# dcjones/polee

Measured on AMD Instinct MI355X. Metric: approx-lik VI iters/sec, higher is better.
Workload: dtype f32

## Files before the change

### include/polee_hip_debug.h

```cpp
#ifndef POLEE_HIP_DEBUG_H
#define POLEE_HIP_DEBUG_H

#include "polee_hip.h"

#ifdef __cplusplus
extern "C" {
#endif

polee_status polee_debug_ptt_plan(const int32_t *node_parent_idxs, const int32_t *node_js, int32_t N,
                                  uint32_t *tour_code, int32_t *tour_tgt, int32_t *leaf_tid,
                                  int32_t *lo, int32_t *mid, int32_t *hi1, int32_t *max_depth);

typedef struct polee_psell_debug polee_psell_debug;
typedef struct {
    int64_t m, n, nnz, num_slices, num_tiles, padded_nnz, num_empty_rows;
    int64_t data_bytes, dict_len;
    int32_t max_row_nnz, max_tile_cols;
    const uint8_t *data;
    const uint32_t *slice_off;
    const uint32_t *tile_slice;
    const uint32_t *tile_dict;
    const uint32_t *dict;
    const uint32_t *row_order;
    const float *slice_ks;
    const uint8_t *slice_flags;
    int64_t num_tiles_a;
    int64_t num_tiles_a1;
    int64_t num_tiles_a1m;
    int64_t num_tiles_a2;
    const uint8_t *slice_w;
    int64_t num_tiles_s;
    int64_t stream_rows[8], stream_nnz[8], stream_bytes[8];
    int64_t csr_num_rows;
    const uint32_t *csr_rowptr;
    const uint32_t *csr_col;
    const float *csr_val;
    const uint32_t *csr_rows;
    int64_t single_num_rows;
    const uint32_t *single_rows;
    const float *single_cnt;
    double single_logsum;
} polee_psell_view;
polee_status polee_debug_psell_build(int64_t m, int64_t n, const void *colptr, int colptr_bytes,
                                     const uint32_t *rowval, const float *nzval,
                                     const int64_t *ks_or_null, polee_psell_debug **out);
polee_status polee_debug_psell_build_device(polee_ctx *ctx, int64_t m, int64_t n, const void *colptr, int colptr_bytes,
                                            const uint32_t *rowval, const float *nzval, const int64_t *ks_or_null,
                                            int device_stages, polee_psell_debug **out);
polee_status polee_debug_psell_view(const polee_psell_debug *p, polee_psell_view *view);
void polee_debug_psell_free(polee_psell_debug *p);

void polee_debug_device_cache_poison(int64_t *checked_blocks, int64_t *bad_blocks, int64_t *bad_words);

polee_status polee_debug_loglik_force_mixed(polee_loglik *ll, int on);

int64_t polee_debug_regression_num_stats(const polee_regression *reg);
polee_status polee_debug_regression_data_pass(polee_regression *reg, const float *noise, float *stats);
polee_status polee_debug_regression_prior_pass(polee_regression *reg, const float *stats, float *loss,
                                               float *grad_or_null);

polee_status polee_debug_comm_allreduce_ms(polee_comm *comm, int64_t count, int32_t reps, double *ms_avg);

polee_status polee_debug_fast_log(polee_ctx *ctx, const double *x, int64_t count, double *out);
polee_status polee_debug_fast_exp(polee_ctx *ctx, const double *x, int64_t count, double *out);

polee_status polee_debug_approx_node_terms(polee_approx *ap, double *tpair, float *bp);

polee_status polee_vi_debug_set_draw_split(polee_vi *vi, int32_t dpw_fwd, int32_t dpw_bwd, int32_t dpw_update);

polee_status polee_debug_gibbs_assignments(polee_gibbs *g, int32_t chain, int32_t *z);

polee_status polee_debug_binomial(polee_ctx *ctx, const int64_t *N, const double *p, int64_t count, uint64_t seed, int64_t *out);

polee_status polee_debug_kmer_edges_count(polee_ctx *ctx_or_null, int64_t n, const uint64_t *sketches, int64_t *count);
polee_status polee_debug_kmer_edges_fill(polee_ctx *ctx_or_null, int64_t n, const uint64_t *sketches, int64_t capacity,
                                         uint32_t *u, uint32_t *v, uint32_t *mat, uint32_t *empt);
polee_status polee_debug_kmer_round_select(polee_ctx *ctx_or_null, int64_t num_nodes, int64_t E, const uint32_t *u, const uint32_t *v,
                                           const uint64_t *key, uint8_t *merged_flags, int32_t *order);

#ifdef __cplusplus
}
#endif
#endif
```

### polee_amd/csrc/debug.cpp

```cpp
#include <algorithm>
#include <memory>

#include "../../include/polee_hip_debug.h"
#include "loglik_internal.hpp"
#include "ptt_internal.hpp"
#include "psell_device.hpp"

using namespace polee;

struct polee_psell_debug {
    PsellHost h;
};

extern "C" {

polee_status polee_debug_ptt_plan(const int32_t *node_parent_idxs, const int32_t *node_js, int32_t N,
                                  uint32_t *tour_code, int32_t *tour_tgt, int32_t *leaf_tid, int32_t *lo,
                                  int32_t *mid, int32_t *hi1, int32_t *max_depth)
{
    if (!node_parent_idxs || !node_js) return fail(nullptr, POLEE_ERR_BAD_ARG, "null argument");
    std::vector<int32_t> l, r, f;
    std::string err = children_from_parents(node_parent_idxs, node_js, N, l, r, f);
    PttPlan pl;
    if (err.empty()) err = build_ptt_plan(l.data(), r.data(), f.data(), N, pl);
// ... 79 lines not shown
        if (needs_host) {
            if (runs_on_device) POLEE_TRY(psell_device_runs_to_host(ctx, DR, R));
            if ((err = psell_stage2(m, n, rowptr.data(), col.data(), val.data(), ks, R, p->h, W)) != "") return bad(err);
        } else {
            rows_on_device = true;
        }
    } else {
        if (runs_on_device) POLEE_TRY(psell_device_runs_to_host(ctx, DR, R));
        if ((err = psell_stage2(m, n, rowptr.data(), col.data(), val.data(), ks, R, p->h, W)) != "") return bad(err);
    }
    if (device_stages & 4) {
        if (!rows_on_device) {
            DW.Nr = W.rows.size();
            DW.npat = W.pat_ptr.size() - 1;
            const size_t b[7] = {0, (size_t)p->h.rows_a1, (size_t)p->h.rows_a1m, (size_t)p->h.rows_a2, (size_t)p->h.rows_a, (size_t)p->h.rows_s, W.rows.size()};
            for (int q = 0; q < 7; ++q) DW.bounds[q] = b[q];
            POLEE_TRY(DW.rows.upload(ctx, W.rows.data(), W.rows.size()));
            POLEE_TRY(DW.run_end.upload(ctx, W.run_end.data(), W.run_end.size()));
            POLEE_TRY(DW.gid.upload(ctx, W.row_gid.data(), W.row_gid.size()));
            POLEE_TRY(DW.form.upload(ctx, W.row_form.data(), W.row_form.size()));
            POLEE_TRY(DW.pat_ptr.upload(ctx, W.pat_ptr.data(), W.pat_ptr.size()));
            POLEE_TRY(DW.pat_col.upload(ctx, W.pat_col.data(), W.pat_col.size()));
        }
        PsellDevOut D;
        POLEE_TRY(psell_device_stage3(ctx, X, DW.view(), p->h, D, true));
    } else {
        if (rows_on_device) POLEE_TRY(psell_device_rows_to_host(ctx, DW, p->h, W));
        if ((err = psell_stage3(m, n, rowptr.data(), col.data(), val.data(), ks, W, p->h)) != "") return bad(err);
    }
    *out = p.release();
    return POLEE_OK;
}

polee_status polee_debug_psell_build(int64_t m, int64_t n, const void *colptr, int colptr_bytes, const uint32_t *rowval,
                                     const float *nzval, const int64_t *ks, polee_psell_debug **out)
{
    return guarded(nullptr, "polee_debug_psell_build", [&] { return debug_psell_build_impl(m, n, colptr, colptr_bytes, rowval, nzval, ks, out); });
}
polee_status polee_debug_psell_build_device(polee_ctx *ctx, int64_t m, int64_t n, const void *colptr, int colptr_bytes,
                                            const uint32_t *rowval, const float *nzval, const int64_t *ks, int device_stages,
                                            polee_psell_debug **out)
{
    return guarded(ctx, "polee_debug_psell_build_device",
                   [&] { return debug_psell_build_device_impl(ctx, m, n, colptr, colptr_bytes, rowval, nzval, ks, device_stages, out); });
}

polee_status polee_debug_psell_view(const polee_psell_debug *p, polee_psell_view *v)
{
    if (!p || !v) return fail(nullptr, POLEE_ERR_BAD_ARG, "null argument");
    const PsellHost &h = p->h;
    v->m = h.m; v->n = h.n; v->nnz = h.nnz;
    v->num_slices = h.num_slices; v->num_tiles = h.num_tiles; v->padded_nnz = h.padded_nnz;
    v->num_empty_rows = h.empty_rows;
    v->data_bytes = (int64_t)h.data.size(); v->dict_len = (int64_t)h.dict.size();
    v->max_row_nnz = h.max_row; v->max_tile_cols = h.max_tile_cols;
    v->data = h.data.data(); v->slice_off = h.slice_off.data(); v->tile_slice = h.tile_slice.data();
    v->tile_dict = h.tile_dict.data(); v->dict = h.dict.data(); v->row_order = h.row_order.data();
    v->slice_ks = h.slice_ks.empty() ? nullptr : h.slice_ks.data();
    v->slice_flags = h.slice_flags.data();
    v->num_tiles_a = h.num_tiles_a;
    v->num_tiles_a1 = h.num_tiles_a1;
    v->num_tiles_a1m = h.num_tiles_a1m;
    v->num_tiles_a2 = h.num_tiles_a2;
    v->num_tiles_s = h.num_tiles_s;
    v->slice_w = h.slice_w.data();
    for (int i = 0; i < 8; ++i) v->stream_rows[i] = v->stream_nnz[i] = v->stream_bytes[i] = 0;
    v->csr_num_rows = (int64_t)h.csr_rows.size();
    v->csr_rowptr = h.csr_rowptr.data();
    v->csr_col = h.csr_col.data();
    v->csr_val = h.csr_val.data();
    v->csr_rows = h.csr_rows.data();
    v->single_num_rows = (int64_t)h.single_rows.size();
    v->single_rows = h.single_rows.data();
    v->single_cnt = h.single_cnt.empty() ? nullptr : h.single_cnt.data();
    v->single_logsum = h.single_logsum;
    for (int i = 0; i < PSELL_NSTREAMS; ++i) {
        v->stream_rows[i] = h.stream_rows[i];
        v->stream_nnz[i] = h.stream_nnz[i];
        v->stream_bytes[i] = h.stream_bytes[i];
    }
    return POLEE_OK;
}

void polee_debug_psell_free(polee_psell_debug *p) { delete p; }

}
```

### polee_amd/csrc/loglik.hip

```cpp
#include "loglik_stream.hpp"

#include <algorithm>
#include <cmath>
#include <queue>

namespace polee {

template <int K>
__device__ inline void scatter_runs(int c, float (&q)[K], float *gw, int lane)
{
    const int c0 = __builtin_amdgcn_readfirstlane(c);
    if (__all(c == c0)) {
        float *gr = gw + c0 * K;
        wave_sum_to_lane63_n<K>(q);
        if (lane == 63) {
#pragma unroll
            for (int k = 0; k < K; ++k) atomicAdd(gr + k, q[k]);
        }
        return;
    }
    const int cprev = __builtin_amdgcn_update_dpp(-1, c, 0x138 , 0xf, 0xf, false);
    const unsigned long long heads = __ballot(c != cprev);
    const unsigned long long upto = lane == 63 ? ~0ull : ((2ull << lane) - 1ull);
    const int dist = lane - (63 - __clzll(heads & upto));
// ... 286 lines not shown
    double ls[PSELL_MAX_K];
#pragma unroll
    for (int k = 0; k < PSELL_MAX_K; ++k) ls[k] = 0.0;
    if (c != 0.0f) {
        const float *xr = x + (size_t)j * K;
        float *gr = g + (size_t)j * K;
#pragma unroll
        for (int k = 0; k < PSELL_MAX_K; ++k)
            if (k < K) {
                const float xv = xr[k];
                if (g) gr[k] += c / xv;
                if (part) ls[k] = (double)c * log((double)xv);
            }
    }
    if (!part) return;
#pragma unroll
    for (int k = 0; k < PSELL_MAX_K; ++k) {
        double v = ls[k];
#pragma unroll
        for (int d = 32; d >= 1; d >>= 1) v += __shfl_down(v, d, 64);
        if ((threadIdx.x & 63) == 0) sm[threadIdx.x >> 6][k] = v;
    }
    __syncthreads();
    if (threadIdx.x < K) part[(size_t)blockIdx.x * K + threadIdx.x] = ((sm[0][threadIdx.x] + sm[1][threadIdx.x]) + sm[2][threadIdx.x]) + sm[3][threadIdx.x];
}
__global__ void single_lp_finish_kernel(const double *__restrict__ part, int nblocks, int K, double logsum, double *__restrict__ lp)
{
    const int k = threadIdx.x;
    if (k >= K) return;
    double s = logsum;
    for (int b = 0; b < nblocks; ++b) s += part[(size_t)b * K + k];
    lp[k] += s;
}

static const double TILE_COST_FIXED[PSELL_NSTREAMS] = {8700.0, 9000.0, 8700.0, 5000.0, 2000.0, 2000.0};
static const double TILE_COST_PER_KIB[PSELL_NSTREAMS] = {350.0, 750.0, 310.0, 1400.0, 3100.0, 3100.0};
static double slices_cost(const PsellHost &h, int stream, uint32_t sa, uint32_t sb)
{
    const double kib = 0.125 * (double)((h.slice_off[sb] & PSELL_OFF_MASK) - (h.slice_off[sa] & PSELL_OFF_MASK));
    static const bool old_cost = getenv("POLEE_OLD_COST") != nullptr;
    if (old_cost) return (kib * 1024.0 + 4096.0) * (stream == PSELL_A2 || stream == PSELL_A2M ? 1.5 : 1.0);
    return TILE_COST_FIXED[stream] + TILE_COST_PER_KIB[stream] * kib;
}
static void wave_cuts(const PsellHost &h, int64_t t, uint32_t s0, uint32_t s1, uint32_t cut[3])
{
    cut[0] = cut[1] = cut[2] = s1;
    if (t >= h.num_tiles_s) return;
    static const bool bytes_cut = getenv("POLEE_BYTES_CUT") != nullptr;
    const int nw = h.stream_of_tile(t) != PSELL_A2M ? 4 : 2;
    static const char *cut_env = getenv("POLEE_CUT_MODEL");
    static double cm[3] = {0, 0, 0};
    static const bool cut_custom = cut_env && sscanf(cut_env, "%lf,%lf,%lf", &cm[0], &cm[1], &cm[2]) == 3;
    auto cost = [&](uint32_t sl) {
        const int w = h.slice_w[sl];
        if (bytes_cut) return 512.0 + 128.0 * (double)((h.slice_off[sl + 1] & PSELL_OFF_MASK) - (h.slice_off[sl] & PSELL_OFF_MASK));
        if (h.stream_of_tile(t) == PSELL_BN) return 6.0 * w + 4.0;
        if (cut_custom) {
            const double ng = (double)((w + 3) / 4);
            const bool cont = (h.slice_flags[sl] & 2) != 0 && sl > s0;
            return cm[0] + cm[1] * ng + (cont ? 0.0 : cm[2] * (1.0 + ng));
        }
        return 4.0 * ((w + 3) / 4) + (w <= 8 ? 8.0 : 16.0 * ((w + 15) / 16)) + 10.0;
    };
    double total = 0.0;
    for (uint32_t sl = s0; sl < s1; ++sl) total += cost(sl);
    double acc = 0.0;
    int wv = 1;
    for (uint32_t sl = s0; sl < s1 && wv < nw; ++sl) {
        acc += cost(sl);
        while (wv < nw && (acc >= total * wv / nw || sl + 1 - (wv == 1 ? s0 : cut[wv - 2]) >= 63u)) cut[wv++ - 1] = sl + 1;
    }
    if (s1 - (nw > 1 ? cut[nw - 2] : s0) > 63u) {
        const uint32_t per = (s1 - s0 + (uint32_t)nw - 1) / (uint32_t)nw;
        for (int q = 1; q < nw; ++q) cut[q - 1] = std::min(s1, s0 + per * (uint32_t)q);
    }
}

void loglik_prepare_tiles(polee_loglik *ll)
{
    const PsellHost &h = ll->host;
    ll->tile_cost.assign((size_t)h.num_tiles, 0.0f);
    for (int64_t t = 0; t < h.num_tiles; ++t)
        ll->tile_cost[(size_t)t] = (float)slices_cost(h, h.stream_of_tile(t), h.tile_slice[t], h.tile_slice[t + 1]);
    ll->tile_cut.assign((size_t)3 * h.num_tiles, 0u);
    for (int64_t t = 0; t < h.num_tiles; ++t) wave_cuts(h, t, h.tile_slice[t], h.tile_slice[t + 1], &ll->tile_cut[(size_t)3 * t]);
}

polee_status loglik_ensure_schedule(polee_loglik *ll, int G)
{
    if (ll->sched_grid == G && ll->d_sched.p) return POLEE_OK;
    const PsellHost &h = ll->host;
    std::vector<uint32_t> order;
    order.reserve((size_t)h.num_tiles_s);
    for (int64_t t = 0; t < h.num_tiles_s; ++t) order.push_back((uint32_t)t);
    std::stable_sort(order.begin(), order.end(), [&](uint32_t a, uint32_t b) { return ll->tile_cost[a] > ll->tile_cost[b]; });
    std::vector<std::vector<uint32_t>> lists((size_t)G);
    {
        typedef std::pair<double, int> Load;
        std::priority_queue<Load, std::vector<Load>, std::greater<Load>> heap;
        for (int b = 0; b < G; ++b) heap.push(Load(0.0, b));
        for (uint32_t t : order) {
            Load l = heap.top();
            heap.pop();
            lists[(size_t)l.second].push_back(t);
            l.first += (double)ll->tile_cost[t];
            heap.push(l);
        }
    }
    size_t rounds = 0;
    for (auto &l : lists) rounds = std::max(rounds, l.size());
    std::vector<PosDesc> sched((rounds + 3) * (size_t)G);
    for (auto &d : sched) {
        d = PosDesc();
        d.tile = POS_NONE;
    }
    for (int b = 0; b < G; ++b) {
        std::vector<uint32_t> big, small;
        for (uint32_t t : lists[b]) (h.stream_of_tile(t) != PSELL_A2 && h.stream_of_tile(t) != PSELL_A2M ? big : small).push_back(t);
        const size_t n = big.size() + small.size();
        size_t ib = 0, is = 0;
        for (size_t j = 0; j < n; ++j) {
            const size_t want = ((j + 1 + (size_t)(b % 3)) * small.size()) / (n + 2);
            const bool take_small = (is < small.size()) && (ib >= big.size() || is < want);
            const uint32_t t = take_small ? small[is++] : big[ib++];
            PosDesc &d = sched[j * (size_t)G + (size_t)b];
            d.tile = t;
            d.s0 = h.tile_slice[t];
            d.s1 = h.tile_slice[t + 1];
            d.d0 = h.tile_dict[t];
            d.L = h.tile_cols[t];
            d.c1 = ll->tile_cut[(size_t)3 * t];
            d.c2 = ll->tile_cut[(size_t)3 * t + 1];
            d.c3 = ll->tile_cut[(size_t)3 * t + 2];
        }
    }
    POLEE_TRY(ll->d_sched.upload(ll->ctx, sched));
    ll->sched_grid = G;
    if (!ll->d_sched_dyn.p) {
        std::vector<uint32_t> dorder(order);
        {
            static const bool plain = getenv("POLEE_DYN_PLAIN_ORDER") != nullptr;
            std::vector<double> key((size_t)h.num_tiles_s, 0.0);
            size_t cnt[PSELL_NSTREAMS] = {}, seen[PSELL_NSTREAMS] = {};
            for (uint32_t t : order) ++cnt[h.stream_of_tile(t)];
            for (uint32_t t : order) {
                const int st = h.stream_of_tile(t);
                key[t] = ((double)seen[st] + 0.5) / (double)cnt[st];
                ++seen[st];
            }
            if (!plain) std::stable_sort(dorder.begin(), dorder.end(), [&](uint32_t a, uint32_t b) { return key[a] < key[b]; });
        }
        std::vector<PosDesc> plist;
        plist.reserve(dorder.size());
        for (size_t i = 0; i < dorder.size(); ++i) {
            const uint32_t t = dorder[i];
            PosDesc d = PosDesc();
            d.tile = t;
            d.s0 = h.tile_slice[t];
            d.s1 = h.tile_slice[t + 1];
            d.d0 = h.tile_dict[t];
            d.L = h.tile_cols[t];
            d.c1 = ll->tile_cut[(size_t)3 * t];
            d.c2 = ll->tile_cut[(size_t)3 * t + 1];
            d.c3 = ll->tile_cut[(size_t)3 * t + 2];
            plist.push_back(d);
        }
        ll->dyn_positions = plist.size();
        std::vector<PosDesc> dynl(plist.size() + (size_t)4 * 4 * 256 + 64);
// ... 346 lines not shown
```

### polee_amd/csrc/loglik_internal.hpp

```cpp
#pragma once
#include "common.hpp"
#include "psell_slice.hpp"

namespace polee {

constexpr int PSELL_MAX_TILE_COLS = 1024;
constexpr int PSELL_TILE_COLS_TARGET = 128;
constexpr int PSELL_DICT_ALIGN = 4;
constexpr int PSELL_TILE_SLICES_A1 = 64;
constexpr int PSELL_TILE_SLICES_A2 = 32;
constexpr int PSELL_TILE_SLICES_B = 16;
constexpr int PSELL_MAX_K = 8;
constexpr int PSELL_NARROW_MAX = 16;
constexpr int PSELL_WIDE_MAX = 32;
constexpr int PSELL_MIXED_NARROW_MAX = 15;
constexpr int PSELL_TILE_SLICES_A2M = 16;
constexpr int PSELL_TILE_SLICES_BN = 64;
constexpr uint32_t PSELL_PACK_CHUNK = 1u << 11;
constexpr uint32_t PSELL_MIXED_SEG_ROWS = 1u << 12;
constexpr double PSELL_PACK_WIDE_RESERVE = 32768.0;
constexpr int PSELL_MIN_UNIFORM_ROWS = 32;
constexpr int PSELL_MIN_UNION_ROWS = 1;

struct PosDesc {
// ... 62 lines not shown
    const uint32_t *csr_col;
    const uint32_t *index_of;
    bool singles_in_g;
};
}

struct polee_xbuild;
namespace polee {
polee_status xbuild_device_view(const polee_xbuild *xb, polee_ctx **ctx, int64_t *rows, int64_t *n, const uint64_t **tcolptr,
                                const uint32_t **trowval, const float **tnzval);
}

struct polee_devx {
    polee_ctx *ctx = nullptr;
    int64_t m = 0, n = 0;
    uint64_t nnz = 0;
    polee::DevBuf<uint64_t> cp;
    polee::DevBuf<uint32_t> rowval;
    polee::DevBuf<float> nzval;
};

struct polee_loglik {
    polee_ctx *ctx = nullptr;
    int refs = 1;
    int64_t m = 0, n = 0, nnz = 0;
    bool has_ks = false;
    bool device_built = false;
    bool force_mixed = false;
    bool xwin_ready = false;
    const double *side_part = nullptr;
    int side_nparts = 0;
    double *side_out = nullptr;
    bool side_done = false;
    polee::PsellHost host;
    polee::DevBuf<uint8_t> d_data;
    polee::DevBuf<uint32_t> d_slice_off, d_tile_slice, d_tile_dict, d_dict;
    polee::DevBuf<float> d_slice_ks;
    polee::DevBuf<uint32_t> d_csr_rowptr;
    polee::DevBuf<uint32_t> d_csr_col;
    polee::DevBuf<float> d_csr_val, d_csr_ks;
    int64_t csr_rows = 0, csr_nnz = 0;
    polee::DevBuf<float> d_single_cnt;
    polee::DevBuf<double> d_single_part;
    bool has_singles = false;
    const polee::LoglikRemap *cur_remap = nullptr;
    polee::DevBuf<float> d_xwin;
    polee::DevBuf<polee::PosDesc> d_sched;
    int sched_grid = 0;
    polee::DevBuf<polee::PosDesc> d_sched_dyn;
    polee::DevBuf<unsigned int> d_dyn_ctr;
    size_t dyn_pad = 0;
    size_t dyn_positions = 0;
    uint32_t dyn_base = 0;
    std::vector<float> tile_cost;
    std::vector<uint32_t> tile_cut;
    int64_t dict_len = 0;
    int occ_cache[polee::PSELL_MAX_K + 1][2][2][2] = {};
    bool deterministic = false;
    polee::DevBuf<float> d_gwin;
    polee::DevBuf<double> d_lpwin;
    polee::DevBuf<uint32_t> d_tslot_ptr, d_tslot, d_theavy;
    polee::DevBuf<float> d_x_rows, d_x_aos, d_g_aos;
    polee::DevBuf<double> d_g_rows, d_lp;
    bool profile = false;
    int prof_every = 1;
    uint64_t prof_tick = 0;
    hipEvent_t cur_e0 = nullptr, cur_e1 = nullptr;
    hipEvent_t cur_p0 = nullptr, cur_p1 = nullptr;
    std::vector<hipEvent_t> prof_events;
    size_t prof_used = 0;
    int64_t prof_launches = 0;
    double prof_ms_total = 0.0, prof_pass_ms_total = 0.0;
    polee_status profile_collect();
};

namespace polee {
void loglik_retain(polee_loglik *ll);
void loglik_release(polee_loglik *ll);
polee_status loglik_eval_device(polee_loglik *ll, const float *d_x, int K, float *d_g, double *d_lp, bool xwin_ready = false,
                                const LoglikRemap *remap = nullptr);
constexpr int SINGLE_THREADS = 256;
constexpr uint32_t GWIN_HEAVY = 32;
void loglik_prepare_tiles(polee_loglik *ll);
polee_status loglik_ensure_schedule(polee_loglik *ll, int G);
std::string csc_to_csr(int64_t m, int64_t n, const void *colptr, int colptr_bytes, const uint32_t *rowval, const float *nzval,
                       BVec<uint64_t> &rowptr, RawVec<uint32_t> &col, RawVec<float> &val);
}
```

### polee_amd/csrc/loglik_stream.hpp

```cpp
#pragma once
#include "loglik_internal.hpp"
#include "wave.hpp"

#include <type_traits>

namespace polee {

typedef float f32x2 __attribute__((ext_vector_type(2)));
typedef float f32x4 __attribute__((ext_vector_type(4)));
typedef const __attribute__((address_space(3))) float *lds_cfp;
typedef __attribute__((address_space(3))) float *lds_fp;
typedef const __attribute__((address_space(3))) f32x2 *lds_cf2p;
typedef const __attribute__((address_space(3))) uint16_t *lds_cu16p;
__device__ inline float lds_f(uint32_t a) { return *reinterpret_cast<lds_cfp>((uintptr_t)a); }

template <int CTRL, int ROW_MASK>
__device__ inline float dpp_mov0(float v)
{
    return __int_as_float(__builtin_amdgcn_update_dpp(0, __float_as_int(v), CTRL, ROW_MASK, 0xf, true));
}

__device__ inline float fast_weight(float ksv, float s)
{
    return s > 0.0f ? ksv * __builtin_amdgcn_rcpf(s) : 0.0f;
// ... 641 lines not shown
{
    constexpr int WMAX = PSELL_NARROW_MAX;
    static_assert(WMAX == 16, "four groups of four transcripts");
    constexpr int KG = (K + 3) / 4;
    const int lane = wave_lane();
    const uint32_t ring_lds = lds_addr(ring);
    const uint32_t xw_lds = lds_addr(xw), gw_lds = lds_addr(gw);
    const int j = lane & 3, b = lane >> 2;
    const uint32_t j4 = 4u * (uint32_t)j;
    uint32_t lc1[4];
#pragma unroll
    for (int u = 0; u < 4; ++u) lc1[u] = ring_lds + ((uint32_t)(lane ^ u) << 2);
    const uint32_t j256 = 256u * (uint32_t)j;

    f32x4 acc[4][KG];
    float xq[8][KG];
#pragma unroll
    for (int g = 0; g < 4; ++g)
#pragma unroll
        for (int kg = 0; kg < KG; ++kg) acc[g][kg] = f32x4{0.f, 0.f, 0.f, 0.f};
#pragma unroll
    for (int t = 0; t < 8; ++t)
#pragma unroll
        for (int kg = 0; kg < KG; ++kg) xq[t][kg] = 0.0f;
    uint32_t xav = aux_lds;
    uint32_t gaq = aux_lds + 32u;
    int pend_w = 0;
    int run_w = 0;
    QuadLp<KG> lp;
    f32x4 floorq = f32x4{ROWSUM_FLOOR, ROWSUM_FLOOR, ROWSUM_FLOOR, ROWSUM_FLOOR};
    asm volatile("" : "+v"(floorq));

    auto flush = [&]() {
        quad_flush_spread<K, 0>(acc[0], gaq, lane, j, dbg);
        if (pend_w > 4) quad_flush_spread<K, 1>(acc[1], gaq, lane, j, dbg);
        if (pend_w > 8) quad_flush_spread<K, 2>(acc[2], gaq, lane, j, dbg);
        if (pend_w > 12) quad_flush_spread<K, 3>(acc[3], gaq, lane, j, dbg);
        pend_w = 0;
    };

    RingCursor<RB, true> rc(ws, ring_lds, extras, lc1[0]);
    uint32_t e_next = (uint32_t)__builtin_amdgcn_readlane((int)ws.ent, 0);
    for (int si = 0; si < ws.nsl; ++si) {
        const uint32_t e0 = e_next;
        const uint32_t e1 = (uint32_t)__builtin_amdgcn_readlane((int)ws.ent, si + 1);
        e_next = e1;
        const SliceEntry se = slice_entry(e0, e1);
        const int flags = se.flags;
        const int nrows = (int)(se.units / 2u) - 1 - (HAS_KS ? 1 : 0);
        int w = MASKED ? run_w : nrows;
        const uint32_t bytes = se.bytes;
        if (!(dbg & 16)) __builtin_amdgcn_s_setprio(3);
        STAMP(1);
        rc.wait_for_steady(bytes);
        STAMP(2);
        if (pend_w != 0 && !(flags & 2)) flush();
        if (pend_w == 0 && !((dbg & 64) && si > 0)) {
            const uint32_t cid = *reinterpret_cast<lds_cu16p>(
                (uintptr_t)(ring_lds + rc.pos_r + (MASKED ? 4u * (uint32_t)(lane & 15) + 2u : 2u * (uint32_t)(lane & 15))));
            const bool live = MASKED ? cid != (uint32_t)PSELL_NO_COL : (lane & 15) < w;
            if (MASKED) {
                run_w = __builtin_popcount((uint32_t)__ballot(live) & 0xffffu);
                w = run_w;
            }
            xav = live ? xw_lds + cid * (uint32_t)(K * 4) : aux_lds;
            gaq = quad_spread_rows(live ? gw_lds + cid * (uint32_t)(K * 4) : aux_lds + 32u, j4);
            quad_load_x_group(xav, 0, j4, xq);
            if (w > 4) quad_load_x_group(xav, 1, j4, xq + 4);
        }
        STAMP(3);

        const uint32_t row0 = wrap_u<RB>(rc.pos_r + 256u);
        f32x4 d1[KG];
        f32x4 kv = f32x4{1.f, 1.f, 1.f, 1.f};
        auto body = [&](auto NGc, auto FASTc) {
            constexpr int NG = decltype(NGc)::value;
            constexpr bool FAST = decltype(FASTc)::value;
            float pv[8], qv[2][4];
            uint32_t bp[4];
            if (FAST) {
#pragma unroll
                for (int u = 0; u < 4; ++u) bp[u] = lc1[u] + rc.pos_r;
            }
            auto read_p = [&](int g0, int g1) {
#pragma unroll
                for (int g = g0; g < g1; ++g) {
                    if (FAST) {
#pragma unroll
                        for (int u = 0; u < 4; ++u) pv[4 * (g - g0) + u] = lds_f(bp[u] + 256u + 1024u * (uint32_t)g + 256u * (uint32_t)u);
                    } else {
                        const uint32_t rg = wrap_u<RB>(row0 + 1024u * (uint32_t)g);
#pragma unroll
                        for (int u = 0; u < 4; ++u) pv[4 * (g - g0) + u] = lds_f(lc1[u] + wrap_u<RB>(rg + 256u * (uint32_t)u));
                    }
                }
            };
            auto read_q = [&](int g0, int g1) {
#pragma unroll
                for (int g = g0; g < g1; ++g) {
                    if (FAST) {
#pragma unroll
                        for (int u = 0; u < 4; ++u) qv[g - g0][u] = lds_f(bp[u] + j256 + 256u + 1024u * (uint32_t)g);
                    } else {
                        const uint32_t rg = wrap_u<RB>(row0 + 1024u * (uint32_t)g);
                        const uint32_t jr = rg + 256u * (uint32_t)j;
                        const uint32_t back = jr >= RB ? RB : 0u;
#pragma unroll
                        for (int u = 0; u < 4; ++u) qv[g - g0][u] = lds_f(lc1[u] + j256 + rg - back);
                    }
                }
            };
            if (HAS_KS)
                kv = *reinterpret_cast<const f32x4 *>(ring + wrap_u<RB>(row0 + 256u * (uint32_t)nrows) + 16u * (uint32_t)b);
            if (MASKED) {
                const uint32_t mk = *reinterpret_cast<lds_cu16p>(
                    (uintptr_t)(lc1[0] + rc.pos_r));
                float mv[4 * NG];
                uint32_t a = lc1[0] + row0;
                const uint32_t lim = lc1[0] + RB;
#pragma unroll
                for (int t = 0; t < 4 * NG; ++t) {
                    mv[t] = lds_f(a);
                    a += ((mk >> t) & 1u) << 8;
                    if (!FAST) a = a >= lim ? a - RB : a;
                }
                slice_consumed([&] { rc.advance(bytes); }, st, dbg);
#pragma unroll
                for (int t = 0; t < 4 * NG; ++t) mv[t] = __uint_as_float(__float_as_uint(mv[t]) & (uint32_t)(((int)(mk << (31 - t))) >> 31));
                quad_phase1_first(d1, floorq, mv, xq);
                if (NG > 1) quad_phase1(d1, mv + 4, xq + 4);
                if (NG > 2) {
                    float xr[8][KG];
                    quad_load_x_group(xav, 2, j4, xr);
                    if (NG > 3) quad_load_x_group(xav, 3, j4, xr + 4);
                    quad_phase1(d1, mv + 8, xr);
                    if (NG > 3) quad_phase1(d1, mv + (NG > 3 ? 12 : 0), xr + 4);
                }
                quad_weights<K, WANT_LP, HAS_KS>(d1, kv, j, lp);
#pragma unroll
                for (int g = 0; g < NG; ++g) {
                    quad_transpose(mv[4 * g], mv[4 * g + 1], mv[4 * g + 2], mv[4 * g + 3]);
                    quad_phase2(acc[g], d1, mv + 4 * g);
                }
            } else if (NG <= 2) {
                read_p(0, NG);
                read_q(0, NG);
                slice_consumed([&] { rc.advance(bytes); }, st, dbg);
                quad_phase1_first(d1, floorq, pv, xq);
                if (NG > 1) quad_phase1(d1, pv + 4, xq + 4);
                quad_weights<K, WANT_LP, HAS_KS>(d1, kv, j, lp);
                quad_phase2(acc[0], d1, qv[0]);
                if (NG > 1) quad_phase2(acc[1], d1, qv[1]);
            } else {
                float pw[8], xr[8][KG], qw[2][4];
                read_p(0, 2);
#pragma unroll
                for (int u = 0; u < 8; ++u) pw[u] = pv[u];
                read_p(2, NG);
                if (!(dbg & 4)) {
                    quad_load_x_group(xav, 2, j4, xr);
                    if (NG > 3) quad_load_x_group(xav, 3, j4, xr + 4);
                } else {
#pragma unroll
                    for (int u = 0; u < 8; ++u)
#pragma unroll
                        for (int kg = 0; kg < KG; ++kg) xr[u][kg] = xq[u][kg];
                }
                asm volatile("s_waitcnt lgkmcnt(0)" ::: "memory");
                if (!(dbg & 16)) __builtin_amdgcn_s_setprio(0);
                quad_phase1_first(d1, floorq, pw, xq);
                quad_phase1(d1, pw + 4, xq + 4);
                quad_phase1(d1, pv, xr);
                if (NG > 3) quad_phase1(d1, pv + 4, xr + 4);
                read_q(0, 2);
#pragma unroll
                for (int u = 0; u < 4; ++u) {
                    qw[0][u] = qv[0][u];
                    qw[1][u] = qv[1][u];
                }
                read_q(2, NG);
                quad_weights<K, WANT_LP, HAS_KS>(d1, kv, j, lp);
                slice_consumed([&] { rc.advance(bytes); }, st, dbg);
                quad_phase2(acc[0], d1, qw[0]);
                quad_phase2(acc[1], d1, qw[1]);
                quad_phase2(acc[2], d1, qv[0]);
                if (NG > 3) quad_phase2(acc[3], d1, qv[1]);
            }
        };
        {
            using std::integral_constant;
            const bool fast = rc.pos_r + bytes <= RB;
            if (fast) {
                if (w <= 4) body(integral_constant<int, 1>(), integral_constant<bool, true>());
                else if (w <= 8) body(integral_constant<int, 2>(), integral_constant<bool, true>());
                else if (w <= 12) body(integral_constant<int, 3>(), integral_constant<bool, true>());
                else body(integral_constant<int, 4>(), integral_constant<bool, true>());
            } else {
                if (w <= 4) body(integral_constant<int, 1>(), integral_constant<bool, false>());
                else if (w <= 8) body(integral_constant<int, 2>(), integral_constant<bool, false>());
                else if (w <= 12) body(integral_constant<int, 3>(), integral_constant<bool, false>());
                else body(integral_constant<int, 4>(), integral_constant<bool, false>());
            }
        }
        pend_w = w;
        STAMP(5);
    }
    if (pend_w != 0) flush();
    if (WANT_LP) quad_lp_reduce<K, HAS_KS>(lp, lane, lpacc);
}

template <int K>
__device__ inline void scatter_runs_lds(int c, float (&q)[K], uint32_t gw_lds, int lane)
{
    auto add = [](uint32_t a, float v) {
        __hip_atomic_fetch_add(reinterpret_cast<lds_fp>((uintptr_t)a), v, __ATOMIC_RELAXED, __HIP_MEMORY_SCOPE_WORKGROUP);
    };
    const int c0 = __builtin_amdgcn_readfirstlane(c);
    if (__all(c == c0)) {
        wave_sum_to_lane63_n<K>(q);
        if (lane == 63) {
#pragma unroll
            for (int k = 0; k < K; ++k) add(gw_lds + (uint32_t)(c0 * K + k) * 4u, q[k]);
        }
        return;
    }
    const int cprev = __builtin_amdgcn_update_dpp(-1, c, 0x138 , 0xf, 0xf, false);
    const unsigned long long heads = __ballot(c != cprev);
    const unsigned long long upto = lane == 63 ? ~0ull : ((2ull << lane) - 1ull);
    const int dist = lane - (63 - __clzll(heads & upto));
    const int rl = lane & 15;
    const float m1 = dist >= 1 ? 1.f : 0.f, m2 = dist >= 2 ? 1.f : 0.f, m4 = dist >= 4 ? 1.f : 0.f,
                m8 = dist >= 8 ? 1.f : 0.f;
    const float mb15 = dist > rl ? 1.f : 0.f;
    const float mb31 = dist > (lane & 31) ? 1.f : 0.f;
#pragma unroll
    for (int k = 0; k < K; ++k) q[k] = fmaf(dpp_mov0<0x111, 0xf>(q[k]), m1, q[k]);
#pragma unroll
    for (int k = 0; k < K; ++k) q[k] = fmaf(dpp_mov0<0x112, 0xf>(q[k]), m2, q[k]);
#pragma unroll
    for (int k = 0; k < K; ++k) q[k] = fmaf(dpp_mov0<0x114, 0xf>(q[k]), m4, q[k]);
#pragma unroll
    for (int k = 0; k < K; ++k) q[k] = fmaf(dpp_mov0<0x118, 0xf>(q[k]), m8, q[k]);
#pragma unroll
    for (int k = 0; k < K; ++k) q[k] = fmaf(dpp_mov0<0x142, 0xa>(q[k]), mb15, q[k]);
#pragma unroll
    for (int k = 0; k < K; ++k) q[k] = fmaf(dpp_mov0<0x143, 0xc>(q[k]), mb31, q[k]);
    const bool tail = lane == 63 || ((heads >> (lane + 1)) & 1ull);
    if (tail) {
#pragma unroll
        for (int k = 0; k < K; ++k)
            if (q[k] != 0.0f) add(gw_lds + (uint32_t)(c * K + k) * 4u, q[k]);
    }
}

template <int K, uint32_t RB, bool WANT_LP, bool HAS_KS>
__device__ inline void mixed_stream(WaveStream &ws, const char *ring, int extras, const float *xw, float *gw, double &lpacc, int dbg, Stamps &st)
{
    const int lane = wave_lane();
    const uint32_t ring_lds = lds_addr(ring);
    const uint32_t xw_lds = lds_addr(xw), gw_lds = lds_addr(gw);
    const uint32_t la4 = ring_lds + 4u * (uint32_t)lane, la2 = ring_lds + 2u * (uint32_t)lane;
    auto x_row_fma = [&](float v, uint32_t c, float (&sacc)[K]) {
        const uint32_t a = xw_lds + c * (uint32_t)(K * 4);
        if constexpr (K % 2 == 0) {
#pragma unroll
            for (int k = 0; k < K / 2; ++k) {
                const f32x2 x = *reinterpret_cast<lds_cf2p>((uintptr_t)(a + 8u * (uint32_t)k));
                sacc[2 * k] = fmaf(v, x.x, sacc[2 * k]);
                sacc[2 * k + 1] = fmaf(v, x.y, sacc[2 * k + 1]);
            }
        } else {
#pragma unroll
            for (int k = 0; k < K; ++k) sacc[k] = fmaf(v, *reinterpret_cast<lds_cfp>((uintptr_t)(a + 4u * (uint32_t)k)), sacc[k]);
        }
    };
    LogAcc lpl[WANT_LP ? K : 1];
    double lp2[WANT_LP ? K : 1];
#pragma unroll
    for (int k = 0; k < (WANT_LP ? K : 1); ++k) {
        lpl[k].init();
        lp2[k] = 0.0;
    }

    uint32_t pos = 0, pos_r = 0;
    for (int si = 0; si < ws.nsl; ++si) {
        const uint32_t e0 = (uint32_t)__builtin_amdgcn_readlane((int)ws.ent, si);
// ... 125 lines not shown
            slice_consumed([&] { stream_advance<RB>(ws, ring_lds, pos, pos_r, bytes); }, st, dbg);
#pragma unroll
            for (int t = 0; t < 16; ++t) mvA[t] = __uint_as_float(__float_as_uint(mvA[t]) & (uint32_t)(((int)(mk << (31 - t))) >> 31));
#pragma unroll
            for (int t = 0; t < 4 * NGH; ++t) mvB[t] = __uint_as_float(__float_as_uint(mvB[t]) & (uint32_t)(((int)(mk << (15 - t))) >> 31));
#pragma unroll
            for (int g = 0; g < 4; g += 2) {
                float xr[8][KG];
                quad_load_x_group(xav0, g, j4, xr);
                quad_load_x_group(xav0, g + 1, j4, xr + 4);
                quad_phase1(d1, mvA + 4 * g, xr);
                quad_phase1(d1, mvA + 4 * g + 4, xr + 4);
            }
#pragma unroll
            for (int g = 0; g < NGH; g += 2) {
                float xr[8][KG];
                quad_load_x_group(xav1, g, j4, xr);
                if (g + 1 < NGH) quad_load_x_group(xav1, g + 1, j4, xr + 4);
                quad_phase1(d1, mvB + 4 * g, xr);
                if (g + 1 < NGH) quad_phase1(d1, mvB + (g + 1 < NGH ? 4 * g + 4 : 0), xr + 4);
            }
            quad_weights<K, WANT_LP, HAS_KS>(d1, kv, j, lp);
#pragma unroll
            for (int g = 0; g < 4; ++g) {
                quad_transpose(mvA[4 * g], mvA[4 * g + 1], mvA[4 * g + 2], mvA[4 * g + 3]);
                quad_phase2(acc[g], d1, mvA + 4 * g);
            }
#pragma unroll
            for (int g = 0; g < 4; ++g) quad_flush_group<K>(acc[g], gav0, g, lane, j, j4, dbg);
#pragma unroll
            for (int g = 0; g < NGH; ++g) {
                quad_transpose(mvB[4 * g], mvB[4 * g + 1], mvB[4 * g + 2], mvB[4 * g + 3]);
                quad_phase2(acc[g], d1, mvB + 4 * g);
            }
#pragma unroll
            for (int g = 0; g < NGH; ++g) quad_flush_group<K>(acc[g], gav1, g, lane, j, j4, dbg);
        };
        {
            using std::integral_constant;
            const bool fast = pos_r + bytes <= RB;
            const int w = run_w;
            if (fast) {
                if (w <= 20) body(integral_constant<int, 1>(), integral_constant<bool, true>());
                else if (w <= 24) body(integral_constant<int, 2>(), integral_constant<bool, true>());
                else if (w <= 28) body(integral_constant<int, 3>(), integral_constant<bool, true>());
                else body(integral_constant<int, 4>(), integral_constant<bool, true>());
            } else {
                if (w <= 20) body(integral_constant<int, 1>(), integral_constant<bool, false>());
                else if (w <= 24) body(integral_constant<int, 2>(), integral_constant<bool, false>());
                else if (w <= 28) body(integral_constant<int, 3>(), integral_constant<bool, false>());
                else body(integral_constant<int, 4>(), integral_constant<bool, false>());
            }
        }
        STAMP(5);
    }
    if (WANT_LP) quad_lp_reduce<K, HAS_KS>(lp, lane, lpacc);
}

#ifdef POLEE_TILE_CYCLES
extern "C" int polee_debug_read_tile_cycles(unsigned long long *tiles, int ntiles, unsigned long long *wgs, int nwgs)
{
    if (hipMemcpyFromSymbol(tiles, HIP_SYMBOL(g_tile_cycles), sizeof(unsigned long long) * (size_t)ntiles) != hipSuccess) return 1;
    if (hipMemcpyFromSymbol(wgs, HIP_SYMBOL(g_wg_cycles), sizeof(unsigned long long) * (size_t)nwgs) != hipSuccess) return 1;
    static unsigned long long z[1 << 17];
    if (hipMemcpyToSymbol(HIP_SYMBOL(g_tile_cycles), z, sizeof(unsigned long long) * (1 << 17)) != hipSuccess) return 1;
    return hipMemcpyToSymbol(HIP_SYMBOL(g_wg_cycles), z, sizeof(unsigned long long) * 4096) == hipSuccess ? 0 : 1;
}
#endif
#ifdef POLEE_STAMPS
extern "C" int polee_debug_read_stamps(unsigned long long *out)
{
    if (hipMemcpyFromSymbol(out, HIP_SYMBOL(g_stamps), sizeof(unsigned long long) * 24) != hipSuccess) return 1;
    unsigned long long z[24] = {0};
    return hipMemcpyToSymbol(HIP_SYMBOL(g_stamps), z, sizeof z) == hipSuccess ? 0 : 1;
}
extern "C" int polee_debug_read_stamps_wave(unsigned long long *out)
{
    if (hipMemcpyFromSymbol(out, HIP_SYMBOL(g_stamps_wave), sizeof(unsigned long long) * 96) != hipSuccess) return 1;
    unsigned long long z[96] = {0};
    return hipMemcpyToSymbol(HIP_SYMBOL(g_stamps_wave), z, sizeof z) == hipSuccess ? 0 : 1;
}
#endif

constexpr uint32_t STREAM_RB1 = 7168u, STREAM_RB2 = 14336u, STREAM_RINGS = 28672u;
template <int K>
constexpr uint32_t stream_ring_total()
{
    return STREAM_RINGS;
}
template <int K>
constexpr uint32_t stream_xw_bytes()
{
    return ((uint32_t)PSELL_TILE_COLS_TARGET * K * 4u + 1023u) & ~1023u;
}
template <int K, bool DET>
constexpr uint32_t stream_lds_bytes()
{
    return stream_ring_total<K>() + (DET ? 6u : 3u) * stream_xw_bytes<K>() + 2u * PSELL_TILE_COLS_TARGET * 4u + 4u * 256u + 2u * 256u + 64u;
}

template <int K, bool WANT_LP, bool HAS_KS, bool DET>
__global__ __launch_bounds__(256) __attribute__((amdgpu_waves_per_eu((WANT_LP || HAS_KS) ? 3 : 4, (WANT_LP || HAS_KS) ? 3 : 4)))
void loglik_stream_kernel(PsellArgs A, int dbg)
{
#ifndef POLEE_ABLATE
    dbg = 0;
#endif
    extern __shared__ float lds[];
    constexpr uint32_t XWB = stream_xw_bytes<K>();
    constexpr uint32_t GWN = DET ? 4u : 1u;
    char *const base = reinterpret_cast<char *>(lds);
    char *const rings = base;
    auto xw_of = [&](int b) -> float * { return reinterpret_cast<float *>(base + stream_ring_total<K>() + (uint32_t)b * XWB); };
    float *const gw = reinterpret_cast<float *>(base + stream_ring_total<K>() + 2 * XWB);
    auto ids_of = [&](int b) -> uint32_t * {
        return reinterpret_cast<uint32_t *>(base + stream_ring_total<K>() + (2 + GWN) * XWB + (uint32_t)b * (PSELL_TILE_COLS_TARGET * 4));
    };
    uint32_t *const entb = reinterpret_cast<uint32_t *>(base + stream_ring_total<K>() + (2 + GWN) * XWB + 2 * PSELL_TILE_COLS_TARGET * 4);
    uint32_t *const descb = entb + 4 * 64;
    float *const auxz = reinterpret_cast<float *>(descb + 2 * 64);

    const int wave = __builtin_amdgcn_readfirstlane(threadIdx.x >> 6);
    const uint32_t G = gridDim.x;
    const bool dyn = A.dyn_ctr != nullptr;
    const PosDesc *__restrict__ sched = dyn ? A.sched_dyn : A.sched;
    uint32_t p2 = blockIdx.x + 2u * G;
    const uint8_t *__restrict__ xwin_b = reinterpret_cast<const uint8_t *>(A.xwin);
    Stamps st;
#ifdef POLEE_STAMPS
    unsigned long long n_slices = 0, n_tiles = 0;
#endif
#ifdef POLEE_TILE_CYCLES
    const unsigned long long t_wg0 = __builtin_amdgcn_s_memtime();
    unsigned long long t_tile0 = t_wg0;
#endif

    auto kind_of = [&](uint32_t tile) -> int { return (int)tile < A.tiles_a1 ? 0 : ((int)tile < A.tiles_a1m ? 2 : ((int)tile < A.tiles_a2 ? 1 : ((int)tile < A.tiles_a ? 3 : 4))); };
    auto share = [&](int kind, const PosDesc &t, uint32_t &sb, uint32_t &se) {
        const int nw = kind == 3 ? 2 : 4;
        uint32_t a1 = t.c1, a2 = t.c2, a3 = t.c3;
        asm volatile("" : "+s"(a1), "+s"(a2), "+s"(a3));
        const uint32_t lo = wave == 0 ? t.s0 : (wave == 1 ? a1 : (wave == 2 ? a2 : a3));
        const uint32_t hi = wave + 1 >= nw ? t.s1 : (wave == 0 ? a1 : (wave == 1 ? a2 : a3));
        sb = wave < nw ? lo : t.s1;
        se = wave < nw ? hi : t.s1;
    };
    auto prefetch = [&](const PosDesc &t, int buf) -> int {
        int cnt = 0;
        const int npx = (int)((t.L * (uint32_t)K * 4u + 1023u) >> 10);
        const uint8_t *src = xwin_b + (size_t)t.d0 * K * 4;
        const uint32_t dst = lds_addr(xw_of(buf));
        for (int p = wave; p < npx; p += 4) {
            dma_1k_keep(uniform_ptr(src + (size_t)p * 1024), (uint32_t)wave_lane() * 16u, dst + (uint32_t)p * 1024u);
            ++cnt;
        }
        if ((uint32_t)wave * 64u < t.L) {
            dma_256(uniform_ptr(A.dict + t.d0 + (uint32_t)wave * 64u), min((uint32_t)wave_lane(), t.L - 1u - (uint32_t)wave * 64u) * 4u,
                    lds_addr(ids_of(buf)) + (uint32_t)wave * 256u);
            ++cnt;
        }
        const int kind = kind_of(t.tile);
        {
            uint32_t sb, se;
            share(kind, t, sb, se);
            dma_256(uniform_ptr(A.slice_off + sb), min((uint32_t)wave_lane(), se - sb) * 4u, lds_addr(entb) + (uint32_t)wave * 256u);
            ++cnt;
        }
        return cnt;
    };
    WaveStream ws;
    const int ahead = (dbg >> 8) & 15;
    auto start_ring = [&](const PosDesc &t) {
        const int kind = kind_of(t.tile);
        ws.nsl = 0; ws.npieces = 0; ws.issued = 0; ws.slot = 0u; ws.primed = 0; ws.ent = 0u; ws.gsrc = A.data;
        uint32_t sb, se;
        share(kind, t, sb, se);
        ws.ent = entb[wave * 64 + wave_lane()];
        ws.nsl = (int)(se - sb);
        const uint32_t cb = (uint32_t)__builtin_amdgcn_readlane((int)ws.ent, 0) & PSELL_OFF_MASK;
        const uint32_t ce = (uint32_t)__builtin_amdgcn_readlane((int)ws.ent, ws.nsl) & PSELL_OFF_MASK;
        ws.npieces = (int)(((ce - cb) * 128u + 1023u) >> 10);
        ws.gsrc = reinterpret_cast<const uint8_t *>(uniform_ptr(A.data + (size_t)cb * 128));
        if (kind != 3) {
            ring_refill<STREAM_RB1>(ws, lds_addr(rings + wave * STREAM_RB1), min(ws.npieces, ahead ? min(ahead, (int)(STREAM_RB1 / 1024u)) : (int)(STREAM_RB1 / 1024u)));
        } else {
            ring_refill<STREAM_RB2>(ws, lds_addr(rings + (wave < 2 ? wave : 0) * STREAM_RB2), min(ws.npieces, ahead ? min(2 * ahead, (int)(STREAM_RB2 / 1024u)) : (int)(STREAM_RB2 / 1024u)));
        }
        ws.primed = ws.issued;
    };

    double lp_a = 0.0;

    PosDesc cur = sched[blockIdx.x];
    if (cur.tile == POS_NONE) return;
    PosDesc nxt = sched[blockIdx.x + G];
    for (int i = threadIdx.x; i < (int)(GWN * XWB / 4u); i += 256) gw[i] = 0.0f;
    for (int i = threadIdx.x; i < (int)(stream_ring_total<K>() / 16u); i += 256)
        reinterpret_cast<float4 *>(rings)[i] = make_float4(0.f, 0.f, 0.f, 0.f);
    if (threadIdx.x < 16) auxz[threadIdx.x] = 0.0f;
    lds_barrier();
    (void)prefetch(cur, 0);
// ... 151 lines not shown
```

Measured before the change: 2777.

## Place x/gradient windows before ring so wrapped reads skip per-row modulo

Reorders the LDS layout so one x window and the gradient windows sit in front of the ring buffers. Ring reads that wrap can then address a contiguous region before the ring instead of computing a wrap per row. The slow (non-FAST) read paths now pick one side offset per group when every row falls on one side of the seam, and fall back to a per-row select otherwise. This removes the per-row modulo arithmetic in the wrapped case, at the cost of more complex LDS addressing and a possibly larger LDS footprint. It also adds a debug export for the wave cuts and census macros.

```diff
diff --git a/include/polee_hip_debug.h b/include/polee_hip_debug.h
--- a/include/polee_hip_debug.h
+++ b/include/polee_hip_debug.h
@@ -48,6 +48,7 @@
                                             const uint32_t *rowval, const float *nzval, const int64_t *ks_or_null,
                                             int device_stages, polee_psell_debug **out);
 polee_status polee_debug_psell_view(const polee_psell_debug *p, polee_psell_view *view);
+polee_status polee_debug_psell_wave_cuts(const polee_psell_debug *p, uint32_t *cuts);
 void polee_debug_psell_free(polee_psell_debug *p);
 
 void polee_debug_device_cache_poison(int64_t *checked_blocks, int64_t *bad_blocks, int64_t *bad_words);
diff --git a/polee_amd/csrc/debug.cpp b/polee_amd/csrc/debug.cpp
--- a/polee_amd/csrc/debug.cpp
+++ b/polee_amd/csrc/debug.cpp
@@ -185,6 +185,17 @@
     return POLEE_OK;
 }
 
+polee_status polee_debug_psell_wave_cuts(const polee_psell_debug *p, uint32_t *cuts)
+{
+    if (!p || !cuts) return fail(nullptr, POLEE_ERR_BAD_ARG, "null argument");
+    return guarded(nullptr, "polee_debug_psell_wave_cuts", [&] {
+        std::vector<uint32_t> c;
+        loglik_tile_cuts(p->h, c);
+        std::copy(c.begin(), c.end(), cuts);
+        return POLEE_OK;
+    });
+}
+
 void polee_debug_psell_free(polee_psell_debug *p) { delete p; }
 
 }
diff --git a/polee_amd/csrc/loglik.hip b/polee_amd/csrc/loglik.hip
--- a/polee_amd/csrc/loglik.hip
+++ b/polee_amd/csrc/loglik.hip
@@ -392,8 +392,12 @@
     ll->tile_cost.assign((size_t)h.num_tiles, 0.0f);
     for (int64_t t = 0; t < h.num_tiles; ++t)
         ll->tile_cost[(size_t)t] = (float)slices_cost(h, h.stream_of_tile(t), h.tile_slice[t], h.tile_slice[t + 1]);
-    ll->tile_cut.assign((size_t)3 * h.num_tiles, 0u);
-    for (int64_t t = 0; t < h.num_tiles; ++t) wave_cuts(h, t, h.tile_slice[t], h.tile_slice[t + 1], &ll->tile_cut[(size_t)3 * t]);
+    loglik_tile_cuts(h, ll->tile_cut);
+}
+void loglik_tile_cuts(const PsellHost &h, std::vector<uint32_t> &cut)
+{
+    cut.assign((size_t)3 * h.num_tiles, 0u);
+    for (int64_t t = 0; t < h.num_tiles; ++t) wave_cuts(h, t, h.tile_slice[t], h.tile_slice[t + 1], &cut[(size_t)3 * t]);
 }
 
 polee_status loglik_ensure_schedule(polee_loglik *ll, int G)
diff --git a/polee_amd/csrc/loglik_internal.hpp b/polee_amd/csrc/loglik_internal.hpp
--- a/polee_amd/csrc/loglik_internal.hpp
+++ b/polee_amd/csrc/loglik_internal.hpp
@@ -168,6 +168,7 @@
 constexpr int SINGLE_THREADS = 256;
 constexpr uint32_t GWIN_HEAVY = 32;
 void loglik_prepare_tiles(polee_loglik *ll);
+void loglik_tile_cuts(const PsellHost &h, std::vector<uint32_t> &cut);
 polee_status loglik_ensure_schedule(polee_loglik *ll, int G);
 std::string csc_to_csr(int64_t m, int64_t n, const void *colptr, int colptr_bytes, const uint32_t *rowval, const float *nzval,
                        BVec<uint64_t> &rowptr, RawVec<uint32_t> &col, RawVec<float> &val);
diff --git a/polee_amd/csrc/loglik_stream.hpp b/polee_amd/csrc/loglik_stream.hpp
--- a/polee_amd/csrc/loglik_stream.hpp
+++ b/polee_amd/csrc/loglik_stream.hpp
@@ -747,36 +747,67 @@
 #pragma unroll
                 for (int u = 0; u < 4; ++u) bp[u] = lc1[u] + rc.pos_r;
             }
+            const uint32_t qs = FAST ? 0u : (uint32_t)__builtin_amdgcn_readfirstlane((int)(((RB - rc.pos_r) >> 8) - 1u));
+            const uint32_t pos_b = FAST ? 0u : (uint32_t)__builtin_amdgcn_readfirstlane((int)(rc.pos_r - RB));
+#ifdef POLEE_CENSUS_SEAM
+            auto one_side = [&](int g0, int g1) { return (POLEE_CENSUS_SEAM) == 0; };
+#else
+            auto one_side = [&](int g0, int g1) { return qs <= 4u * (uint32_t)g0 || qs >= 4u * (uint32_t)g1; };
+#endif
             auto read_p = [&](int g0, int g1) {
-#pragma unroll
-                for (int g = g0; g < g1; ++g) {
-                    if (FAST) {
+                if (FAST) {
+#pragma unroll
+                    for (int g = g0; g < g1; ++g)
 #pragma unroll
                         for (int u = 0; u < 4; ++u) pv[4 * (g - g0) + u] = lds_f(bp[u] + 256u + 1024u * (uint32_t)g + 256u * (uint32_t)u);
-                    } else {
-                        const uint32_t rg = wrap_u<RB>(row0 + 1024u * (uint32_t)g);
-#pragma unroll
-                        for (int u = 0; u < 4; ++u) pv[4 * (g - g0) + u] = lds_f(lc1[u] + wrap_u<RB>(rg + 256u * (uint32_t)u));
-                    }
+                } else if (one_side(g0, g1)) {
+                    const uint32_t side = qs <= 4u * (uint32_t)g0 ? pos_b : rc.pos_r;
+#pragma unroll
+                    for (int u = 0; u < 4; ++u) bp[u] = lc1[u] + side;
+#pragma unroll
+                    for (int g = g0; g < g1; ++g)
+#pragma unroll
+                        for (int u = 0; u < 4; ++u) pv[4 * (g - g0) + u] = lds_f(bp[u] + 256u + 1024u * (uint32_t)g + 256u * (uint32_t)u);
+                } else {
+#pragma unroll
+                    for (int g = g0; g < g1; ++g)
+#pragma unroll
+                        for (int u = 0; u < 4; ++u) {
+                            const uint32_t side = qs > (uint32_t)(4 * g + u) ? rc.pos_r : pos_b;
+                            pv[4 * (g - g0) + u] = lds_f(lc1[u] + side + (256u + 1024u * (uint32_t)g + 256u * (uint32_t)u));
+                        }
+                    asm volatile("");
                 }
             };
             auto read_q = [&](int g0, int g1) {
-#pragma unroll
-                for (int g = g0; g < g1; ++g) {
-                    if (FAST) {
+                if (FAST) {
+#pragma unroll
+                    for (int g = g0; g < g1; ++g)
 #pragma unroll
                         for (int u = 0; u < 4; ++u) qv[g - g0][u] = lds_f(bp[u] + j256 + 256u + 1024u * (uint32_t)g);
-                    } else {
-                        const uint32_t rg = wrap_u<RB>(row0 + 1024u * (uint32_t)g);
-                        const uint32_t jr = rg + 256u * (uint32_t)j;
-                        const uint32_t back = jr >= RB ? RB : 0u;
-#pragma unroll
-                        for (int u = 0; u < 4; ++u) qv[g - g0][u] = lds_f(lc1[u] + j256 + rg - back);
+                } else if (one_side(g0, g1)) {
+                    const uint32_t side = qs <= 4u * (uint32_t)g0 ? pos_b : rc.pos_r;
+#pragma unroll
+                    for (int u = 0; u < 4; ++u) bp[u] = lc1[u] + side;
+#pragma unroll
+                    for (int g = g0; g < g1; ++g)
+#pragma unroll
+                        for (int u = 0; u < 4; ++u) qv[g - g0][u] = lds_f(bp[u] + j256 + 256u + 1024u * (uint32_t)g);
+                } else {
+                    uint32_t jr = j256;
+                    asm volatile("" : "+v"(jr));
+#pragma unroll
+                    for (int g = g0; g < g1; ++g) {
+                        const uint32_t side = jr + ((int)jr < (int)((qs << 8) - 1024u * (uint32_t)g) ? rc.pos_r : pos_b);
+#pragma unroll
+                        for (int u = 0; u < 4; ++u) qv[g - g0][u] = lds_f(lc1[u] + side + (256u + 1024u * (uint32_t)g));
                     }
+                    asm volatile("");
                 }
             };
-            if (HAS_KS)
-                kv = *reinterpret_cast<const f32x4 *>(ring + wrap_u<RB>(row0 + 256u * (uint32_t)nrows) + 16u * (uint32_t)b);
+            if (HAS_KS) {
+                kv = *reinterpret_cast<const f32x4 *>(ring + ((FAST ? rc.pos_r : pos_b) + 256u + 256u * (uint32_t)nrows) + 16u * (uint32_t)b);
+            }
             if (MASKED) {
                 const uint32_t mk = *reinterpret_cast<lds_cu16p>(
                     (uintptr_t)(lc1[0] + rc.pos_r));
@@ -852,6 +883,9 @@
                 if (NG > 3) quad_phase2(acc[3], d1, qv[1]);
             }
         };
+#ifdef POLEE_CENSUS_BODY
+        body(std::integral_constant<int, (POLEE_CENSUS_BODY) / 2 + 1>(), std::integral_constant<bool, ((POLEE_CENSUS_BODY) & 1) != 0>());
+#else
         {
             using std::integral_constant;
             const bool fast = rc.pos_r + bytes <= RB;
@@ -867,6 +901,7 @@
                 else body(integral_constant<int, 4>(), integral_constant<bool, false>());
             }
         }
+#endif
         pend_w = w;
         STAMP(5);
     }
@@ -1158,6 +1193,7 @@
 }
 #endif
 
+constexpr uint32_t STREAM_RING_MIN = 5120u;
 constexpr uint32_t STREAM_RB1 = 7168u, STREAM_RB2 = 14336u, STREAM_RINGS = 28672u;
 template <int K>
 constexpr uint32_t stream_ring_total()
@@ -1170,9 +1206,15 @@
     return ((uint32_t)PSELL_TILE_COLS_TARGET * K * 4u + 1023u) & ~1023u;
 }
 template <int K, bool DET>
+constexpr uint32_t stream_ring_base()
+{
+    return (DET ? 5u : 2u) * stream_xw_bytes<K>() > STREAM_RING_MIN ? (DET ? 5u : 2u) * stream_xw_bytes<K>() : STREAM_RING_MIN;
+}
+template <int K, bool DET>
 constexpr uint32_t stream_lds_bytes()
 {
-    return stream_ring_total<K>() + (DET ? 6u : 3u) * stream_xw_bytes<K>() + 2u * PSELL_TILE_COLS_TARGET * 4u + 4u * 256u + 2u * 256u + 64u;
+    static_assert(STREAM_RING_MIN >= 256u * (PSELL_NARROW_MAX + 1) && STREAM_RING_MIN % 1024u == 0u, "see above");
+    return stream_ring_base<K, DET>() + stream_ring_total<K>() + stream_xw_bytes<K>() + 2u * PSELL_TILE_COLS_TARGET * 4u + 4u * 256u + 2u * 256u + 64u;
 }
 
 template <int K, bool WANT_LP, bool HAS_KS, bool DET>
@@ -1186,13 +1228,14 @@
     constexpr uint32_t XWB = stream_xw_bytes<K>();
     constexpr uint32_t GWN = DET ? 4u : 1u;
     char *const base = reinterpret_cast<char *>(lds);
-    char *const rings = base;
-    auto xw_of = [&](int b) -> float * { return reinterpret_cast<float *>(base + stream_ring_total<K>() + (uint32_t)b * XWB); };
-    float *const gw = reinterpret_cast<float *>(base + stream_ring_total<K>() + 2 * XWB);
-    auto ids_of = [&](int b) -> uint32_t * {
-        return reinterpret_cast<uint32_t *>(base + stream_ring_total<K>() + (2 + GWN) * XWB + (uint32_t)b * (PSELL_TILE_COLS_TARGET * 4));
-    };
-    uint32_t *const entb = reinterpret_cast<uint32_t *>(base + stream_ring_total<K>() + (2 + GWN) * XWB + 2 * PSELL_TILE_COLS_TARGET * 4);
+    constexpr uint32_t RING0 = stream_ring_base<K, DET>();
+    static_assert(RING0 >= (1u + GWN) * XWB && RING0 % 1024u == 0u, "x window 1 and the gradient windows lie in front of the rings");
+    constexpr uint32_t TAIL0 = RING0 + stream_ring_total<K>() + XWB;
+    char *const rings = base + RING0;
+    auto xw_of = [&](int b) -> float * { return reinterpret_cast<float *>(base + (b ? 0u : RING0 + stream_ring_total<K>())); };
+    float *const gw = reinterpret_cast<float *>(base + XWB);
+    auto ids_of = [&](int b) -> uint32_t * { return reinterpret_cast<uint32_t *>(base + TAIL0 + (uint32_t)b * (PSELL_TILE_COLS_TARGET * 4)); };
+    uint32_t *const entb = reinterpret_cast<uint32_t *>(base + TAIL0 + 2 * PSELL_TILE_COLS_TARGET * 4);
     uint32_t *const descb = entb + 4 * 64;
     float *const auxz = reinterpret_cast<float *>(descb + 2 * 64);
 
```

Result: no change. 2783, median of 6 (+0.2%).
